# qradiolink/qradiolink

Measured on AMD Instinct MI355X. Metric: IQ MSamples/sec through RX demod chain, higher is better.
Workload: dtype f32

## Files before the change

### qradiolink_amd/csrc/kernels_ff.hip

```cpp
#include "devmath.hpp"
#include "engine.hpp"
#include <cstdlib>

namespace qrl {

__device__ __forceinline__ float2 ringc_at(const RingC& r, int b, int64_t i)
{
    if (i < 0) return make_float2(0.f, 0.f);
    return r.p[(size_t)b * (r.mask + 1u) + ((uint32_t)i & r.mask)];
}
__device__ __forceinline__ float ringf_at(const RingF& r, int b, int64_t i)
{
    if (i < 0) return 0.f;
    return r.p[(size_t)b * (r.mask + 1u) + ((uint32_t)i & r.mask)];
}

__global__ __launch_bounds__(256) void k_fir_ccf(const FirCcfParams P)
{
    const int b = blockIdx.y;
    const uint32_t t = blockIdx.x * 256u + threadIdx.x;
    if (t >= P.count) return;
    if (t == 0 && P.counts) P.counts[b * 4 + 0] = P.count;
    const int64_t n = (int64_t)(P.q0 + t);
    float ar = 0.f, ai = 0.f;
    for (int k = 0; k < P.nt; ++k) {
        const float h = P.taps[k];
        const float2 x = ringc_at(P.in, b, n - k);
        ar = fmaf(h, x.x, ar);
        ai = fmaf(h, x.y, ai);
    }
    const float2 y = make_float2(ar, ai);
    P.out.p[(size_t)b * (P.out.mask + 1u) + ((uint32_t)n & P.out.mask)] = y;
    if (P.port && t < P.port_cap) P.port[(size_t)b * P.port_cap + t] = y;
}
constexpr int FT_R = 4, FT_OUT = 256 * FT_R, FT_MAXT = 1024;

template <int MAXT>
__global__ __launch_bounds__(256) void k_fir_ccf_tiled(const FirCcfParams P)
{
    __shared__ float taps[MAXT];
    __shared__ float2 xs[FT_OUT + MAXT];
    const int b = blockIdx.y, tid = threadIdx.x;
    const uint32_t t0 = blockIdx.x * (uint32_t)FT_OUT;
    const int nt = P.nt;
    for (int k = tid; k < nt; k += 256) taps[k] = P.taps[k];
    const int64_t first = (int64_t)(P.q0 + t0) - (nt - 1);
    const int span = min((uint32_t)FT_OUT, P.count - t0) + nt - 1;
    for (int i = tid; i < span; i += 256) xs[i] = ringc_at(P.in, b, first + i);
    __syncthreads();
    if (blockIdx.x == 0 && tid == 0 && P.counts) P.counts[b * 4 + 0] = P.count;
    float ar[FT_R], ai[FT_R];
#pragma unroll
    for (int r = 0; r < FT_R; ++r) { ar[r] = 0.f; ai[r] = 0.f; }
    const float2* xp = xs + (nt - 1) + tid;
    for (int k = 0; k < nt; ++k) {
        const float h = taps[k];
#pragma unroll
        for (int r = 0; r < FT_R; ++r) {
            const float2 x = xp[256 * r - k];
            ar[r] = fmaf(h, x.x, ar[r]);
            ai[r] = fmaf(h, x.y, ai[r]);
        }
    }
#pragma unroll
    for (int r = 0; r < FT_R; ++r) {
        const uint32_t t = t0 + tid + 256u * r;
        if (t < P.count) {
            const int64_t n = (int64_t)(P.q0 + t);
            const float2 y = make_float2(ar[r], ai[r]);
            P.out.p[(size_t)b * (P.out.mask + 1u) + ((uint32_t)n & P.out.mask)] = y;
            if (P.port && t < P.port_cap) P.port[(size_t)b * P.port_cap + t] = y;
        }
    }
}
__global__ __launch_bounds__(256) void k_fir_fff_tiled(const FirFffParams P)
{
    __shared__ float taps[FT_MAXT];
    __shared__ float xs[FT_OUT + FT_MAXT];
    const int b = blockIdx.y, tid = threadIdx.x;
    const uint32_t t0 = blockIdx.x * (uint32_t)FT_OUT;
    const int nt = P.nt;
    for (int k = tid; k < nt; k += 256) taps[k] = P.taps[k];
    const int64_t first = (int64_t)(P.q0 + t0) - (nt - 1);
    const int span = min((uint32_t)FT_OUT, P.count - t0) + nt - 1;
    for (int i = tid; i < span; i += 256) xs[i] = ringf_at(P.in, b, first + i);
    __syncthreads();
    float a[FT_R];
#pragma unroll
    for (int r = 0; r < FT_R; ++r) a[r] = 0.f;
    const float* xp = xs + (nt - 1) + tid;
    for (int k = 0; k < nt; ++k) {
        const float h = taps[k];
#pragma unroll
        for (int r = 0; r < FT_R; ++r) a[r] = fmaf(h, xp[256 * r - k], a[r]);
    }
#pragma unroll
    for (int r = 0; r < FT_R; ++r) {
        const uint32_t t = t0 + tid + 256u * r;
        if (t < P.count) P.out.p[(size_t)b * (P.out.mask + 1u) + ((uint32_t)(P.q0 + t) & P.out.mask)] = a[r];
    }
}
static bool fir_use_tiled(int nt, uint32_t count) { return nt >= 8 && nt <= FT_MAXT && count >= 512; }

void launch_fir_ccf(const FirCcfParams& p, int batch, hipStream_t s)
{
    if (!p.count) return;
    if (fir_use_tiled(p.nt, p.count)) hipLaunchKernelGGL(k_fir_ccf_tiled<FT_MAXT>, dim3((p.count + FT_OUT - 1) / FT_OUT, batch), dim3(256), 0, s, p);
    else if (p.nt > FT_MAXT && p.nt <= 2 * FT_MAXT && p.count >= 512)
        hipLaunchKernelGGL(k_fir_ccf_tiled<2 * FT_MAXT>, dim3((p.count + FT_OUT - 1) / FT_OUT, batch), dim3(256), 0, s, p);
    else hipLaunchKernelGGL(k_fir_ccf, dim3((p.count + 255) / 256, batch), dim3(256), 0, s, p);
}

__global__ __launch_bounds__(256) void k_fir_fff(const FirFffParams P)
{
    const int b = blockIdx.y;
    const uint32_t t = blockIdx.x * 256u + threadIdx.x;
    if (t >= P.count) return;
    const int64_t n = (int64_t)(P.q0 + t);
    float a = 0.f;
    for (int k = 0; k < P.nt; ++k) a = fmaf(P.taps[k], ringf_at(P.in, b, n - k), a);
    P.out.p[(size_t)b * (P.out.mask + 1u) + ((uint32_t)n & P.out.mask)] = a;
}
void launch_fir_fff(const FirFffParams& p, int batch, hipStream_t s)
{
    if (!p.count) return;
    if (fir_use_tiled(p.nt, p.count)) hipLaunchKernelGGL(k_fir_fff_tiled, dim3((p.count + FT_OUT - 1) / FT_OUT, batch), dim3(256), 0, s, p);
    else hipLaunchKernelGGL(k_fir_fff, dim3((p.count + 255) / 256, batch), dim3(256), 0, s, p);
}

__global__ __launch_bounds__(256) void k_quad_demod(const QuadDemodParams P)
{
    __shared__ float T[257];
    for (int k = threadIdx.x; k < 257; k += 256) T[k] = P.atan_tab[k];
    __syncthreads();
    const int b = blockIdx.y;
    const uint32_t t = blockIdx.x * 256u + threadIdx.x;
    if (t >= P.count) return;
    const int64_t n = (int64_t)(P.q0 + t);
    const float2 a = ringc_at(P.in, b, n), p = ringc_at(P.in, b, n - 1);
    const float re = a.x * p.x + a.y * p.y;
    const float im = a.y * p.x - a.x * p.y;
    const float ang = fast_atan2f_lut(im, re, T);
    P.out.p[(size_t)b * (P.out.mask + 1u) + ((uint32_t)n & P.out.mask)] = P.gain * ang;
    if (P.out2.p) P.out2.p[(size_t)b * (P.out2.mask + 1u) + ((uint32_t)n & P.out2.mask)] = P.gain2 * ang;
    if (P.s16) {
        float r = rintf(((P.gain * ang) * P.s16_level) * P.s16_scale);
        if (r > 32767.0f) r = 32767.0f;
        if (r < -32768.0f) r = -32768.0f;
        if (t < P.s16_cap) P.s16[(size_t)b * P.s16_cap + t] = (int16_t)r;
        if (t == 0 && P.s16_counts) P.s16_counts[b] = P.count < P.s16_cap ? P.count : (uint32_t)P.s16_cap;
    }
}
void launch_quad_demod(const QuadDemodParams& p, int batch, hipStream_t s)
{
    if (!p.count) return;
    hipLaunchKernelGGL(k_quad_demod, dim3((p.count + 255) / 256, batch), dim3(256), 0, s, p);
}

__global__ __launch_bounds__(256) void k_disc_2fsk(const Disc2fskParams P)
{
    const int b = blockIdx.y;
    const uint32_t t = blockIdx.x * 256u + threadIdx.x;
    if (t >= P.count) return;
    const int64_t n = (int64_t)(P.q0 + t);
    float ar = 0.f, ai = 0.f, br = 0.f, bi = 0.f;
    for (int k = 0; k < P.nt; ++k) {
        const float2 x = ringc_at(P.in, b, n - k);
        const float2 h = P.up[k];
        ar = fmaf(h.x, x.x, ar); ai = fmaf(h.x, x.y, ai);
        br = fmaf(h.y, x.x, br); bi = fmaf(h.y, x.y, bi);
    }
    const float ur = ar - bi, ui = ai + br, lr = ar + bi, li = ai - br;
    const float mu = sqrtf(ur * ur + ui * ui);
    const float ml = sqrtf(lr * lr + li * li);
    float r = mu / ml;
    if (!(r >= 0.0f)) r = 0.0f;
    if (r > 2.0f) r = 2.0f;
    P.out.p[(size_t)b * (P.out.mask + 1u) + ((uint32_t)n & P.out.mask)] = r + (-1.0f);
}
__global__ __launch_bounds__(256) void k_disc_4fsk(const Disc4fskParams P)
{
    const int b = blockIdx.y;
    const uint32_t t = blockIdx.x * 256u + threadIdx.x;
    if (t >= P.count) return;
    const int64_t n = (int64_t)(P.q0 + t);
    float re[4] = {0.f, 0.f, 0.f, 0.f}, im[4] = {0.f, 0.f, 0.f, 0.f};
    for (int k = 0; k < P.nt; ++k) {
        const float2 x = ringc_at(P.in, b, n - k);
#pragma unroll
        for (int q = 0; q < 4; ++q) {
            const float2 h = P.taps[q * P.nt + k];
            re[q] = fmaf(h.x, x.x, re[q]); re[q] = fmaf(-h.y, x.y, re[q]);
            im[q] = fmaf(h.x, x.y, im[q]); im[q] = fmaf(h.y, x.x, im[q]);
        }
    }
    const float m1 = sqrtf(re[0] * re[0] + im[0] * im[0]), m2 = sqrtf(re[1] * re[1] + im[1] * im[1]);
    const float m3 = sqrtf(re[2] * re[2] + im[2] * im[2]), m4 = sqrtf(re[3] * re[3] + im[3] * im[3]);
    const float A = 0.707107f;
    float2 v = make_float2(0.f, 0.f);
    if (m1 > m2 && m1 > m3 && m1 > m4) v = make_float2(-A, -A);
    else if (m2 > m1 && m2 > m3 && m2 > m4) v = make_float2(-A, A);
    else if (m3 > m2 && m3 > m1 && m3 > m4) v = make_float2(A, A);
    else if (m4 > m2 && m4 > m1 && m4 > m3) v = make_float2(A, -A);
    P.out.p[(size_t)b * (P.out.mask + 1u) + ((uint32_t)n & P.out.mask)] = v;
}
void launch_disc_4fsk(const Disc4fskParams& p, int batch, hipStream_t s)
{
    if (!p.count) return;
    hipLaunchKernelGGL(k_disc_4fsk, dim3((p.count + 255) / 256, batch), dim3(256), 0, s, p);
}

void launch_disc_2fsk(const Disc2fskParams& p, int batch, hipStream_t s)
{
    if (!p.count) return;
    hipLaunchKernelGGL(k_disc_2fsk, dim3((p.count + 255) / 256, batch), dim3(256), 0, s, p);
}

constexpr int FF_PL = 280, FF_PF = 264, FF_PD = 264;

template <int PITCH, int NQ, typename TapT, typename ItemT, typename Fma>
__device__ __forceinline__ void ff_window4(const ItemT* __restrict__ tile, int w, int nq_rt, const TapT* __restrict__ taps, Fma&& fma4)
{
    ItemT cur[4], nxt[4];
#pragma unroll
    for (int s = 0; s < 4; ++s) cur[s] = tile[s * PITCH + w];
    auto quad = [&](int q) {
        --w;
#pragma unroll
        for (int s = 0; s < 4; ++s) nxt[s] = tile[s * PITCH + w];
        const TapT h0 = taps[4 * q], h1 = taps[4 * q + 1], h2 = taps[4 * q + 2], h3 = taps[4 * q + 3];
        fma4(h0, cur[0], cur[1], cur[2], cur[3]);
        fma4(h1, nxt[3], cur[0], cur[1], cur[2]);
        fma4(h2, nxt[2], nxt[3], cur[0], cur[1]);
        fma4(h3, nxt[1], nxt[2], nxt[3], cur[0]);
#pragma unroll
        for (int s = 0; s < 4; ++s) cur[s] = nxt[s];
    };
    if constexpr (NQ > 0) {
#pragma unroll 4
        for (int q = 0; q < NQ; ++q) quad(q);
    } else {
        for (int q = 0; q < nq_rt; ++q) quad(q);
    }
}

template <int NQF, int NQB, int NQS>
__global__ __launch_bounds__(256) void k_2fsk_ff(const Fsk2FfParams P)
{
    __shared__ float2 lt[4 * FF_PL];
    __shared__ float2 ft[4 * FF_PF];
    __shared__ float dt[4 * FF_PD];
    const int b = blockIdx.y, tid = threadIdx.x;
    const int hf = P.nf - 1, hb = P.nb - 1, hs = P.ns - 1;
    const int T = 1024 - hb - hs;
    const int64_t n0t = (int64_t)P.q0 + (int64_t)blockIdx.x * T;
    const int nl = 1024 + hf, nd = T + hs;
    if (tid < 4) { lt[tid * FF_PL] = make_float2(0.f, 0.f); ft[tid * FF_PF] = make_float2(0.f, 0.f); dt[tid * FF_PD] = 0.f; }
    {
        float2 v[5];
#pragma unroll
        for (int it = 0; it < 5; ++it) {
            const int64_t a = n0t - (hf + hb + hs) + tid + 256 * it;
            v[it] = P.in.p[(size_t)b * (P.in.mask + 1u) + ((uint32_t)a & P.in.mask)];
            if (a < 0) v[it] = make_float2(0.f, 0.f);
        }
#pragma unroll
        for (int it = 0; it < 5; ++it) {
            const int i = tid + 256 * it;
            if (i < nl) lt[(i & 3) * FF_PL + (i >> 2) + 1] = v[it];
        }
    }
    __syncthreads();
    {
        float2 a[4] = {{0.f, 0.f}, {0.f, 0.f}, {0.f, 0.f}, {0.f, 0.f}};
        ff_window4<FF_PL, NQF>(lt, tid + (hf >> 2) + 1, (hf >> 2) + 1, P.tf,
                          [&](float h, const float2& x0, const float2& x1, const float2& x2, const float2& x3) {
                              a[0].x = fmaf(h, x0.x, a[0].x); a[0].y = fmaf(h, x0.y, a[0].y);
                              a[1].x = fmaf(h, x1.x, a[1].x); a[1].y = fmaf(h, x1.y, a[1].y);
                              a[2].x = fmaf(h, x2.x, a[2].x); a[2].y = fmaf(h, x2.y, a[2].y);
                              a[3].x = fmaf(h, x3.x, a[3].x); a[3].y = fmaf(h, x3.y, a[3].y);
                          });
#pragma unroll
        for (int r = 0; r < 4; ++r) {
            const bool neg = n0t - (hb + hs) + 4 * tid + r < 0;
            ft[r * FF_PF + tid + 1] = neg ? make_float2(0.f, 0.f) : a[r];
        }
    }
    __syncthreads();
    if (4 * tid < nd) {
        float ar[4] = {0.f, 0.f, 0.f, 0.f}, ai[4] = {0.f, 0.f, 0.f, 0.f}, br[4] = {0.f, 0.f, 0.f, 0.f}, bi[4] = {0.f, 0.f, 0.f, 0.f};
        const int nq = NQB > 0 ? NQB : (hb >> 2) + 1;
        int w = tid + (hb >> 2) + 1;
        float2 cur[4], nxt[4];
#pragma unroll
        for (int s = 0; s < 4; ++s) cur[s] = ft[s * FF_PF + w];
        auto step = [&](const float2 h, const float2& x0, const float2& x1, const float2& x2, const float2& x3) {
            const float2 xs[4] = {x0, x1, x2, x3};
#pragma unroll
            for (int r = 0; r < 4; ++r) {
                ar[r] = fmaf(h.x, xs[r].x, ar[r]); ai[r] = fmaf(h.x, xs[r].y, ai[r]);
                br[r] = fmaf(h.y, xs[r].x, br[r]); bi[r] = fmaf(h.y, xs[r].y, bi[r]);
            }
        };
        auto quad = [&](int q) {
            --w;
#pragma unroll
            for (int s = 0; s < 4; ++s) nxt[s] = ft[s * FF_PF + w];
            step(P.up[4 * q], cur[0], cur[1], cur[2], cur[3]);
            step(P.up[4 * q + 1], nxt[3], cur[0], cur[1], cur[2]);
            step(P.up[4 * q + 2], nxt[2], nxt[3], cur[0], cur[1]);
            step(P.up[4 * q + 3], nxt[1], nxt[2], nxt[3], cur[0]);
#pragma unroll
            for (int s = 0; s < 4; ++s) cur[s] = nxt[s];
        };
        if constexpr (NQB > 0) {
#pragma unroll 4
            for (int q = 0; q < NQB; ++q) quad(q);
        } else {
            for (int q = 0; q < nq; ++q) quad(q);
        }
#pragma unroll
        for (int r = 0; r < 4; ++r) {
            const float ur = ar[r] - bi[r], ui = ai[r] + br[r], lr = ar[r] + bi[r], li = ai[r] - br[r];
            const float mu = sqrtf(ur * ur + ui * ui);
            const float ml = sqrtf(lr * lr + li * li);
            float v = mu / ml;
            if (!(v >= 0.0f)) v = 0.0f;
            if (v > 2.0f) v = 2.0f;
            dt[r * FF_PD + tid + 1] = (n0t - hs + 4 * tid + r < 0) ? 0.f : v + (-1.0f);
        }
    }
    __syncthreads();
    if (4 * tid < T) {
        float a[4] = {0.f, 0.f, 0.f, 0.f};
        ff_window4<FF_PD, NQS>(dt, tid + (hs >> 2) + 1, (hs >> 2) + 1, P.ts,
                          [&](float h, float x0, float x1, float x2, float x3) {
                              a[0] = fmaf(h, x0, a[0]); a[1] = fmaf(h, x1, a[1]); a[2] = fmaf(h, x2, a[2]); a[3] = fmaf(h, x3, a[3]);
                          });
        const uint32_t t0 = blockIdx.x * (uint32_t)T + 4u * tid;
        if (t0 == 0 && P.counts) P.counts[b * 4 + 0] = P.count;
        const int wf = tid + ((hb + hs) >> 2) + 1;
#pragma unroll
        for (int r = 0; r < 4; ++r) {
            const uint32_t t = t0 + r;
            if (t < P.count) {
                const int64_t n = n0t + 4 * tid + r;
                P.out.p[(size_t)b * (P.out.mask + 1u) + ((uint32_t)n & P.out.mask)] = a[r];
                if (P.port && t < P.port_cap) P.port[(size_t)b * P.port_cap + t] = ft[r * FF_PF + wf];
            }
        }
    }
}
int fsk2_ff_padded(int n) { return (n - 1 + 3) / 4 * 4 + 1; }
void launch_2fsk_ff(const Fsk2FfParams& p, int batch, hipStream_t s)
{
    if (!p.count) return;
    const int T = 1024 - (p.nb - 1) - (p.ns - 1);
    const dim3 grid((p.count + T - 1) / T, batch);
    static const bool rt = [] { const char* e = getenv("QRL_FF_RUNTIME_TAPS"); return e && atoi(e) != 0; }();
    const int qf = (p.nf - 1) / 4 + 1, qb = (p.nb - 1) / 4 + 1, qs = (p.ns - 1) / 4 + 1;
    if (!rt && qf == 11 && qb == 11 && qs == 7) hipLaunchKernelGGL((k_2fsk_ff<11, 11, 7>), grid, dim3(256), 0, s, p);
    else hipLaunchKernelGGL((k_2fsk_ff<0, 0, 0>), grid, dim3(256), 0, s, p);
}

}
```

Baseline: 536,500.

## Add MFMA-based fused 2FSK filter chain kernel for fixed tap counts

Adds a new kernel that computes the three FIR stages of the 2FSK fused demod (lowpass, complex bandpass pair, symbol filter) as matrix ops using 16x16x4 f32 MFMA instructions. Samples go into a transposed shared-memory image, taps are staged in shared memory, and DPP swaps recombine the real and imaginary parts. It also drops the compile-time tap-count template specialisation from the scalar fallback kernel, so that path now loops over runtime tap counts. The MFMA kernel is used only when the tap counts match 41/41/25, which adds complexity and layout risk.

```diff
diff --git a/qradiolink_amd/csrc/kernels_ff.hip b/qradiolink_amd/csrc/kernels_ff.hip
--- a/qradiolink_amd/csrc/kernels_ff.hip
+++ b/qradiolink_amd/csrc/kernels_ff.hip
@@ -218,8 +218,8 @@
 
 constexpr int FF_PL = 280, FF_PF = 264, FF_PD = 264;
 
-template <int PITCH, int NQ, typename TapT, typename ItemT, typename Fma>
-__device__ __forceinline__ void ff_window4(const ItemT* __restrict__ tile, int w, int nq_rt, const TapT* __restrict__ taps, Fma&& fma4)
+template <int PITCH, typename TapT, typename ItemT, typename Fma>
+__device__ __forceinline__ void ff_window4(const ItemT* __restrict__ tile, int w, int nq, const TapT* __restrict__ taps, Fma&& fma4)
 {
     ItemT cur[4], nxt[4];
 #pragma unroll
@@ -236,15 +236,9 @@
 #pragma unroll
         for (int s = 0; s < 4; ++s) cur[s] = nxt[s];
     };
-    if constexpr (NQ > 0) {
-#pragma unroll 4
-        for (int q = 0; q < NQ; ++q) quad(q);
-    } else {
-        for (int q = 0; q < nq_rt; ++q) quad(q);
-    }
-}
-
-template <int NQF, int NQB, int NQS>
+    for (int q = 0; q < nq; ++q) quad(q);
+}
+
 __global__ __launch_bounds__(256) void k_2fsk_ff(const Fsk2FfParams P)
 {
     __shared__ float2 lt[4 * FF_PL];
@@ -273,7 +267,7 @@
     __syncthreads();
     {
         float2 a[4] = {{0.f, 0.f}, {0.f, 0.f}, {0.f, 0.f}, {0.f, 0.f}};
-        ff_window4<FF_PL, NQF>(lt, tid + (hf >> 2) + 1, (hf >> 2) + 1, P.tf,
+        ff_window4<FF_PL>(lt, tid + (hf >> 2) + 1, (hf >> 2) + 1, P.tf,
                           [&](float h, const float2& x0, const float2& x1, const float2& x2, const float2& x3) {
                               a[0].x = fmaf(h, x0.x, a[0].x); a[0].y = fmaf(h, x0.y, a[0].y);
                               a[1].x = fmaf(h, x1.x, a[1].x); a[1].y = fmaf(h, x1.y, a[1].y);
@@ -289,7 +283,7 @@
     __syncthreads();
     if (4 * tid < nd) {
         float ar[4] = {0.f, 0.f, 0.f, 0.f}, ai[4] = {0.f, 0.f, 0.f, 0.f}, br[4] = {0.f, 0.f, 0.f, 0.f}, bi[4] = {0.f, 0.f, 0.f, 0.f};
-        const int nq = NQB > 0 ? NQB : (hb >> 2) + 1;
+        const int nq = (hb >> 2) + 1;
         int w = tid + (hb >> 2) + 1;
         float2 cur[4], nxt[4];
 #pragma unroll
@@ -313,12 +307,7 @@
 #pragma unroll
             for (int s = 0; s < 4; ++s) cur[s] = nxt[s];
         };
-        if constexpr (NQB > 0) {
-#pragma unroll 4
-            for (int q = 0; q < NQB; ++q) quad(q);
-        } else {
-            for (int q = 0; q < nq; ++q) quad(q);
-        }
+        for (int q = 0; q < nq; ++q) quad(q);
 #pragma unroll
         for (int r = 0; r < 4; ++r) {
             const float ur = ar[r] - bi[r], ui = ai[r] + br[r], lr = ar[r] + bi[r], li = ai[r] - br[r];
@@ -333,7 +322,7 @@
     __syncthreads();
     if (4 * tid < T) {
         float a[4] = {0.f, 0.f, 0.f, 0.f};
-        ff_window4<FF_PD, NQS>(dt, tid + (hs >> 2) + 1, (hs >> 2) + 1, P.ts,
+        ff_window4<FF_PD>(dt, tid + (hs >> 2) + 1, (hs >> 2) + 1, P.ts,
                           [&](float h, float x0, float x1, float x2, float x3) {
                               a[0] = fmaf(h, x0, a[0]); a[1] = fmaf(h, x1, a[1]); a[2] = fmaf(h, x2, a[2]); a[3] = fmaf(h, x3, a[3]);
                           });
@@ -351,6 +340,162 @@
         }
     }
 }
+constexpr int FM_NF = 41, FM_NB = 41, FM_NS = 25;
+constexpr int FM_HF = FM_NF - 1, FM_HB = FM_NB - 1, FM_HS = FM_NS - 1;
+constexpr int FM_T = 1024 - FM_HB - FM_HS;
+constexpr int FM_NL = 1024 + FM_HF;
+constexpr int FM_M1 = (FM_NF + 15 + 3) / 4, FM_M2 = (FM_NB + 15 + 3) / 4, FM_M3 = (FM_NS + 15 + 3) / 4;
+constexpr int FM_TP = 15 + 3 + 4 * FM_M1;
+constexpr int FM_C0 = 4;
+constexpr int FM_P = 72, FM_PD = 80;
+static_assert((FM_NL - 1) / 16 + FM_C0 < FM_P && (1008 + 15 + FM_HS) / 16 + FM_C0 < FM_PD, "image pitch");
+static_assert(16 * FM_PD <= 2 * 16 * FM_P, "d image aliases the staged items");
+typedef float f32x4_ff __attribute__((ext_vector_type(4)));
+__device__ __forceinline__ int fm_pos(int i, int pitch) { return (i & 15) * pitch + (i >> 4) + FM_C0; }
+__device__ __forceinline__ float fm_swap_pair(float v) { return __int_as_float(__builtin_amdgcn_mov_dpp(__float_as_int(v), 0xB1, 0xF, 0xF, false)); }
+
+__global__ __launch_bounds__(256) void k_2fsk_ff_mfma(const Fsk2FfParams P)
+{
+    __shared__ __align__(16) float lt[2 * 16 * FM_P];
+    __shared__ __align__(16) float ft[2 * 16 * FM_P];
+    __shared__ float tpf[FM_TP], tpa[FM_TP], tpb[FM_TP], tps[FM_TP];
+    float* const dt = lt;
+    const int b = blockIdx.y, tid = threadIdx.x, lane = tid & 63;
+    const int wv = __builtin_amdgcn_readfirstlane(tid >> 6);
+    const int col = lane & 15, kk = lane >> 4, cmp = col & 1, nl = col >> 1;
+    const int64_t n0t = (int64_t)P.q0 + (int64_t)blockIdx.x * FM_T;
+    const int64_t a_end = (int64_t)P.q0 + P.count;
+    if (tid < FM_TP) {
+        const int k = tid - 15;
+        const float2 u = (k >= 0 && k < FM_NB) ? P.up[k] : make_float2(0.f, 0.f);
+        tpf[tid] = (k >= 0 && k < FM_NF) ? P.tf[k] : 0.f;
+        tpa[tid] = u.x; tpb[tid] = u.y;
+        tps[tid] = (k >= 0 && k < FM_NS) ? P.ts[k] : 0.f;
+    }
+    const int tbase = col + kk;
+    {
+        const int c = ((tid >> 1) & 7) | ((tid >> 7) << 3), r = (tid & 1) | (((tid >> 4) & 7) << 1);
+        float2 v[5];
+#pragma unroll
+        for (int it = 0; it < 5; ++it) {
+            const int64_t a = n0t - (FM_HF + FM_HB + FM_HS) + 256 * it + 16 * c + r;
+            v[it] = P.in.p[(size_t)b * (P.in.mask + 1u) + ((uint32_t)a & P.in.mask)];
+            if (a < 0 || a >= a_end) v[it] = make_float2(0.f, 0.f);
+        }
+#pragma unroll
+        for (int it = 0; it < 5; ++it) {
+            const int i = 256 * it + 16 * c + r;
+            if (i < FM_NL) reinterpret_cast<float2*>(lt)[fm_pos(i, FM_P)] = v[it];
+        }
+        if (tid < FM_HF) reinterpret_cast<float2*>(ft)[fm_pos(1024 + tid, FM_P)] = make_float2(0.f, 0.f);
+    }
+    __syncthreads();
+    constexpr int QC = (FM_M1 - 1) >> 2;
+    static_assert(FM_M2 == FM_M1, "stages 1 and 2 share the walk");
+    {
+        float hf[FM_M1];
+#pragma unroll
+        for (int m = 0; m < FM_M1; ++m) hf[m] = tpf[tbase + 4 * m];
+        f32x4_ff acc[2];
+        int ob[2][4];
+#pragma unroll
+        for (int c = 0; c < 2; ++c) {
+            const int it0 = FM_HF + 16 * (8 * (wv + 4 * c) + nl) + 15 - kk;
+#pragma unroll
+            for (int j = 0; j < 4; ++j) ob[c][j] = 2 * (fm_pos(it0 - 4 * j, FM_P) - QC) + cmp;
+            acc[c] = f32x4_ff{0.f, 0.f, 0.f, 0.f};
+        }
+#pragma unroll
+        for (int m = 0; m < FM_M1; ++m)
+#pragma unroll
+            for (int c = 0; c < 2; ++c)
+                acc[c] = __builtin_amdgcn_mfma_f32_16x16x4f32(hf[m], lt[ob[c][m & 3] + 2 * (QC - (m >> 2))], acc[c], 0, 0, 0);
+#pragma unroll
+        for (int c = 0; c < 2; ++c) {
+            const int n = 8 * (wv + 4 * c) + nl;
+#pragma unroll
+            for (int r = 0; r < 4; ++r) {
+                const int j = 16 * n + 4 * kk + r;
+                ft[2 * fm_pos(j, FM_P) + cmp] = (n0t - (FM_HB + FM_HS) + j < 0) ? 0.f : acc[c][r];
+            }
+        }
+    }
+    __syncthreads();
+    {
+        float ha[FM_M2], hb[FM_M2];
+#pragma unroll
+        for (int m = 0; m < FM_M2; ++m) { ha[m] = tpa[tbase + 4 * m]; hb[m] = tpb[tbase + 4 * m]; }
+        f32x4_ff aa[2], ab[2];
+        int ob[2][4];
+#pragma unroll
+        for (int c = 0; c < 2; ++c) {
+            const int it0 = FM_HB + 16 * (8 * (wv + 4 * c) + nl) + 15 - kk;
+#pragma unroll
+            for (int j = 0; j < 4; ++j) ob[c][j] = 2 * (fm_pos(it0 - 4 * j, FM_P) - QC) + cmp;
+            aa[c] = f32x4_ff{0.f, 0.f, 0.f, 0.f}; ab[c] = aa[c];
+        }
+#pragma unroll
+        for (int m = 0; m < FM_M2; ++m)
+#pragma unroll
+            for (int c = 0; c < 2; ++c) {
+                const float x = ft[ob[c][m & 3] + 2 * (QC - (m >> 2))];
+                aa[c] = __builtin_amdgcn_mfma_f32_16x16x4f32(ha[m], x, aa[c], 0, 0, 0);
+                ab[c] = __builtin_amdgcn_mfma_f32_16x16x4f32(hb[m], x, ab[c], 0, 0, 0);
+            }
+#pragma unroll
+        for (int c = 0; c < 2; ++c) {
+            const int n = 8 * (wv + 4 * c) + nl;
+#pragma unroll
+            for (int h = 0; h < 2; ++h) {
+                const int r = cmp ? 3 - h : h;
+                const float sa = fm_swap_pair(cmp ? aa[c][h] : aa[c][3 - h]), sb = fm_swap_pair(cmp ? ab[c][h] : ab[c][3 - h]);
+                const float oa = cmp ? aa[c][3 - h] : aa[c][h], obb = cmp ? ab[c][3 - h] : ab[c][h];
+                const float ar = cmp ? sa : oa, ai = cmp ? oa : sa, br = cmp ? sb : obb, bi = cmp ? obb : sb;
+                const float ur = ar - bi, ui = ai + br, lr = ar + bi, li = ai - br;
+                const float mu = sqrtf(ur * ur + ui * ui);
+                const float ml = sqrtf(lr * lr + li * li);
+                float v = mu / ml;
+                if (!(v >= 0.0f)) v = 0.0f;
+                if (v > 2.0f) v = 2.0f;
+                const int j = 16 * n + 4 * kk + r;
+                dt[fm_pos(j, FM_PD)] = (n0t - FM_HS + j < 0) ? 0.f : v + (-1.0f);
+            }
+        }
+    }
+    __syncthreads();
+    if (blockIdx.x == 0 && tid == 0 && P.counts) P.counts[b * 4 + 0] = P.count;
+    {
+        constexpr int QS = (FM_M3 - 1) >> 2;
+        float hs[FM_M3];
+#pragma unroll
+        for (int m = 0; m < FM_M3; ++m) hs[m] = tps[tbase + 4 * m];
+        const int n = 16 * wv + col;
+        const int it0 = FM_HS + 16 * n + 15 - kk;
+        int ob[4];
+#pragma unroll
+        for (int j = 0; j < 4; ++j) ob[j] = fm_pos(it0 - 4 * j, FM_PD) - QS;
+        f32x4_ff acc = {0.f, 0.f, 0.f, 0.f};
+#pragma unroll
+        for (int m = 0; m < FM_M3; ++m) acc = __builtin_amdgcn_mfma_f32_16x16x4f32(hs[m], dt[ob[m & 3] + QS - (m >> 2)], acc, 0, 0, 0);
+        float* orow = P.out.p + (size_t)b * (P.out.mask + 1u);
+#pragma unroll
+        for (int r = 0; r < 4; ++r) {
+            const int o = 16 * n + 4 * kk + r;
+            const uint32_t t = blockIdx.x * (uint32_t)FM_T + (uint32_t)o;
+            if (o < FM_T && t < P.count) orow[(uint32_t)(n0t + o) & P.out.mask] = acc[r];
+        }
+    }
+    if (P.port) {
+#pragma unroll
+        for (int k = 0; k < (FM_T + 255) / 256; ++k) {
+            const int o = tid + 256 * k;
+            const uint32_t t = blockIdx.x * (uint32_t)FM_T + (uint32_t)o;
+            if (o < FM_T && t < P.count && t < P.port_cap)
+                P.port[(size_t)b * P.port_cap + t] = reinterpret_cast<const float2*>(ft)[fm_pos(FM_HB + FM_HS + o, FM_P)];
+        }
+    }
+}
+
 int fsk2_ff_padded(int n) { return (n - 1 + 3) / 4 * 4 + 1; }
 void launch_2fsk_ff(const Fsk2FfParams& p, int batch, hipStream_t s)
 {
@@ -358,9 +503,8 @@
     const int T = 1024 - (p.nb - 1) - (p.ns - 1);
     const dim3 grid((p.count + T - 1) / T, batch);
     static const bool rt = [] { const char* e = getenv("QRL_FF_RUNTIME_TAPS"); return e && atoi(e) != 0; }();
-    const int qf = (p.nf - 1) / 4 + 1, qb = (p.nb - 1) / 4 + 1, qs = (p.ns - 1) / 4 + 1;
-    if (!rt && qf == 11 && qb == 11 && qs == 7) hipLaunchKernelGGL((k_2fsk_ff<11, 11, 7>), grid, dim3(256), 0, s, p);
-    else hipLaunchKernelGGL((k_2fsk_ff<0, 0, 0>), grid, dim3(256), 0, s, p);
-}
-
-}
+    if (!rt && p.nf == FM_NF && p.nb == FM_NB && p.ns == FM_NS) hipLaunchKernelGGL(k_2fsk_ff_mfma, grid, dim3(256), 0, s, p);
+    else hipLaunchKernelGGL(k_2fsk_ff, grid, dim3(256), 0, s, p);
+}
+
+}
```

Result: slower. 523,100, median of 2 (-2.5%).
